# Improbable-AI/walk-these-ways

Hardware: AMD Instinct MI355X
Metric: env-steps/sec (sim+PPO) (higher is better)
Workload: dtype f32

## Files before the change

### walk-these-ways_amd/csrc/go1ppo_gemm.h

```cpp
#pragma once

#define GEMM_BM 128
#define GEMM_BN 128
#define GEMM_BK 64

typedef __attribute__((address_space(3))) void lds_void_t;
typedef __attribute__((address_space(1))) const void global_cvoid_t;

__device__ __forceinline__ void glds16(const bf16_t* g, bf16_t* lds_wave_base) {
  __builtin_amdgcn_global_load_lds((global_cvoid_t*)g, (lds_void_t*)lds_wave_base, 16, 0, 0);
}

template <int EPI>
__device__ __forceinline__ void gemm_nt_body(const Go1PpoGemmArgs& a, bf16_t (*lds)[2][GEMM_BM * GEMM_BK]) {
  const int lane = threadIdx.x & 63, wave = threadIdx.x >> 6;
  const int nwg = gridDim.x, orig = blockIdx.x;
  const int q = nwg >> 3, r = nwg & 7, xcd = orig & 7;
  const int logical = (xcd < r ? xcd * (q + 1) : r * (q + 1) + (xcd - r) * q) + (orig >> 3);
  const int tiles_n = (a.N + GEMM_BN - 1) / GEMM_BN;
  const int m0 = (logical / tiles_n) * GEMM_BM, n0 = (logical % tiles_n) * GEMM_BN;

  const int srow = lane >> 3;
  const bf16_t* ga[4];
  const bf16_t* gb[4];
#pragma unroll
  for (int p = 0; p < 4; p++) {
    int R = (wave * 4 + p) * 8 + srow;
    int chunk = (lane & 7) ^ ((R >> 1) & 7);
    int ra = m0 + R < a.M ? m0 + R : a.M - 1;
    int rb = n0 + R < a.N ? n0 + R : a.N - 1;
    ga[p] = (const bf16_t*)a.A + (int64_t)ra * a.lda + chunk * 8;
    gb[p] = (const bf16_t*)a.B + (int64_t)rb * a.ldb + chunk * 8;
  }
  auto stage = [&](int buf, int k0) {
#pragma unroll
    for (int p = 0; p < 4; p++) {
      glds16(ga[p] + k0, &lds[buf][0][(wave * 4 + p) * 8 * GEMM_BK]);
      glds16(gb[p] + k0, &lds[buf][1][(wave * 4 + p) * 8 * GEMM_BK]);
    }
  };

  const int fr = lane & 15, fg = lane >> 4;
  int foff[2];
#pragma unroll
  for (int kk = 0; kk < 2; kk++) foff[kk] = fr * GEMM_BK + (((kk * 4 + fg) ^ (fr >> 1)) << 3);
  const int wm = wave >> 1, wn = wave & 1;

  f32x4 acc[4][4];
#pragma unroll
  for (int i = 0; i < 4; i++)
#pragma unroll
    for (int j = 0; j < 4; j++) acc[i][j] = f32x4{0.f, 0.f, 0.f, 0.f};

  const bool wide = !(a.N & 7) && !(a.ldc & 7) && !((uintptr_t)a.C & 15) && (EPI != 2 || (!(a.ldh & 7) && !((uintptr_t)a.H & 15)));
  uint4 hrow[8];
  if (EPI == 2 && wide) {
#pragma unroll
    for (int it = 0; it < 8; it++) {
      int m = m0 + (int)(threadIdx.x >> 4) + 16 * it, n = n0 + (int)(threadIdx.x & 15) * 8;
      m = m < a.M ? m : a.M - 1;
      n = n < a.N ? n : a.N - 8;
      hrow[it] = *reinterpret_cast<const uint4*>((const bf16_t*)a.H + (int64_t)m * a.ldh + n);
    }
  }
  uint2 hpre[4][4];
  if (EPI == 2 && !wide) {
#pragma unroll
    for (int j = 0; j < 4; j++) {
      int n = n0 + wn * 64 + j * 16 + fg * 4;
      n = n < a.N ? n : a.N - 4;
#pragma unroll
      for (int i = 0; i < 4; i++) {
        int m = m0 + wm * 64 + i * 16 + fr;
        m = m < a.M ? m : a.M - 1;
        hpre[j][i] = *reinterpret_cast<const uint2*>((const bf16_t*)a.H + (int64_t)m * a.ldh + n);
      }
    }
  }
  const int KT = a.K / GEMM_BK;
  stage(0, 0);
  for (int kt = 0; kt < KT; kt++) {
    const int buf = kt & 1;
    asm volatile("s_waitcnt vmcnt(0)" ::: "memory");
    __syncthreads();
    if (kt + 1 < KT) stage(buf ^ 1, (kt + 1) * GEMM_BK);
    const bf16_t* la = &lds[buf][0][wm * 64 * GEMM_BK];
    const bf16_t* lb = &lds[buf][1][wn * 64 * GEMM_BK];
#pragma unroll
    for (int kk = 0; kk < 2; kk++) {
      bf16x8_t xa[4], wb[4];
#pragma unroll
      for (int i = 0; i < 4; i++) xa[i] = *reinterpret_cast<const bf16x8_t*>(la + i * 16 * GEMM_BK + foff[kk]);
#pragma unroll
      for (int j = 0; j < 4; j++) wb[j] = *reinterpret_cast<const bf16x8_t*>(lb + j * 16 * GEMM_BK + foff[kk]);
#pragma unroll
      for (int j = 0; j < 4; j++)
#pragma unroll
        for (int i = 0; i < 4; i++) acc[j][i] = __builtin_amdgcn_mfma_f32_16x16x32_bf16(wb[j], xa[i], acc[j][i], 0, 0, 0);
    }
  }

  if (wide) {
    __syncthreads();
    float* img = reinterpret_cast<float*>(&lds[0][0][0]);
#pragma unroll
    for (int j = 0; j < 4; j++) {
      const int nl = wn * 64 + j * 16 + fg * 4, n = n0 + nl;
      f32x4 bias = f32x4{0.f, 0.f, 0.f, 0.f};
      if (a.bias && n < a.N) {
        if (a.bias_bf16) {
          const uint2 braw = *reinterpret_cast<const uint2*>(reinterpret_cast<const bf16_t*>(a.bias) + n);
          bias = f32x4{__uint_as_float(braw.x << 16), __uint_as_float(braw.x & 0xffff0000u), __uint_as_float(braw.y << 16),
                       __uint_as_float(braw.y & 0xffff0000u)};
        } else bias = *reinterpret_cast<const f32x4*>(a.bias + n);
      }
      const bool act = EPI == 1 && n >= a.elu_c0 && n < a.elu_c1 && !(n >= a.elu_skip_c0 && n < a.elu_skip_c1);
#pragma unroll
      for (int i = 0; i < 4; i++) {
        const int row = wm * 64 + i * 16 + fr;
        f32x4 v = acc[j][i] + bias;
        if (act) {
#pragma unroll
          for (int e = 0; e < 4; e++) v[e] = elu1(v[e]);
        }
        *reinterpret_cast<f32x4*>(img + row * 128 + ((((nl >> 2)) ^ (row & 15)) << 2)) = v;
      }
    }
    __syncthreads();
    const int c8 = (int)(threadIdx.x & 15);
    const int n = n0 + c8 * 8;
#pragma unroll
    for (int it = 0; it < 8; it++) {
      const int row = (int)(threadIdx.x >> 4) + 16 * it, m = m0 + row;
      const f32x4 lo = *reinterpret_cast<const f32x4*>(img + row * 128 + (((2 * c8) ^ (row & 15)) << 2));
      const f32x4 hi = *reinterpret_cast<const f32x4*>(img + row * 128 + (((2 * c8 + 1) ^ (row & 15)) << 2));
      float v[8] = {lo[0], lo[1], lo[2], lo[3], hi[0], hi[1], hi[2], hi[3]};
      if (EPI == 2) {
        const uint32_t hw[4] = {hrow[it].x, hrow[it].y, hrow[it].z, hrow[it].w};
#pragma unroll
        for (int e = 0; e < 4; e++) {
          const float h0 = __uint_as_float(hw[e] << 16), h1 = __uint_as_float(hw[e] & 0xffff0000u);
          v[2 * e] *= h0 > 0.f ? 1.f : h0 + 1.f;
          v[2 * e + 1] *= h1 > 0.f ? 1.f : h1 + 1.f;
        }
      }
      if (m < a.M && n < a.N) {
        uint4 o;
        uint32_t* ow = reinterpret_cast<uint32_t*>(&o);
#pragma unroll
        for (int e = 0; e < 4; e++) {
          f32x2 p2 = {v[2 * e], v[2 * e + 1]};
          ow[e] = __builtin_bit_cast(uint32_t, __builtin_convertvector(p2, bf16x2_t));
        }
        *reinterpret_cast<uint4*>((bf16_t*)a.C + (int64_t)m * a.ldc + n) = o;
      }
    }
    return;
  }
#pragma unroll
  for (int j = 0; j < 4; j++) {
    const int n = n0 + wn * 64 + j * 16 + fg * 4;
    if (n >= a.N) continue;
    f32x4 bias = f32x4{0.f, 0.f, 0.f, 0.f};
    if (a.bias) {
      if (a.bias_bf16) {
        const uint2 braw = *reinterpret_cast<const uint2*>(reinterpret_cast<const bf16_t*>(a.bias) + n);
        bias = f32x4{__uint_as_float(braw.x << 16), __uint_as_float(braw.x & 0xffff0000u), __uint_as_float(braw.y << 16),
                     __uint_as_float(braw.y & 0xffff0000u)};
      } else bias = *reinterpret_cast<const f32x4*>(a.bias + n);
    }
#pragma unroll
    for (int i = 0; i < 4; i++) {
      const int m = m0 + wm * 64 + i * 16 + fr;
      if (m >= a.M) continue;
      float v[4];
#pragma unroll
      for (int e = 0; e < 4; e++) v[e] = acc[j][i][e] + bias[e];
      if (EPI == 1) {
        if (n >= a.elu_c0 && n < a.elu_c1 && !(n >= a.elu_skip_c0 && n < a.elu_skip_c1)) {
#pragma unroll
          for (int e = 0; e < 4; e++) v[e] = elu1(v[e]);
        }
      } else if (EPI == 2) {
        const uint2 hraw = hpre[j][i];
        float h[4] = {__uint_as_float(hraw.x << 16), __uint_as_float(hraw.x & 0xffff0000u), __uint_as_float(hraw.y << 16),
                      __uint_as_float(hraw.y & 0xffff0000u)};
#pragma unroll
        for (int e = 0; e < 4; e++) v[e] *= h[e] > 0.f ? 1.f : h[e] + 1.f;
      }
      f32x2 lo = {v[0], v[1]}, hi = {v[2], v[3]};
      uint2 o;
      o.x = __builtin_bit_cast(uint32_t, __builtin_convertvector(lo, bf16x2_t));
      o.y = __builtin_bit_cast(uint32_t, __builtin_convertvector(hi, bf16x2_t));
      *reinterpret_cast<uint2*>((bf16_t*)a.C + (int64_t)m * a.ldc + n) = o;
    }
  }
}

template <int EPI>
__global__ __launch_bounds__(256, 2) void gemm_nt_kernel(Go1PpoGemmArgs a) {
  __shared__ __attribute__((aligned(1024))) bf16_t lds[2][2][GEMM_BM * GEMM_BK];
  gemm_nt_body<EPI>(a, lds);
}
template <int EPI>
__global__ __launch_bounds__(256, 2) void gemm_nt_pair_kernel(Go1PpoGemmArgs a, Go1PpoGemmArgs b) {
  __shared__ __attribute__((aligned(1024))) bf16_t lds[2][2][GEMM_BM * GEMM_BK];
  gemm_nt_body<EPI>(blockIdx.y == 0 ? a : b, lds);
}

static int gemm_nt_check(const Go1PpoGemmArgs* a) {
  if (!a || !a->A || !a->B || !a->C || a->M <= 0 || a->N <= 0 || a->K <= 0) return -1;
  if ((a->K % GEMM_BK) || (a->N & 3) || (a->lda & 7) || (a->ldb & 7) || (a->ldc & 3) || !aligned16(a->A) || !aligned16(a->B) ||
      ((uintptr_t)a->C & 7))
    return -2;
  if (a->epilogue == 2 && (!a->H || (a->ldh & 3) || ((uintptr_t)a->H & 7))) return -3;
  if (a->bias && ((uintptr_t)a->bias & (a->bias_bf16 ? 7 : 15))) return -4;
  return 0;
}

extern "C" int go1ppo_gemm_nt_pair(const Go1PpoGemmArgs* a, const Go1PpoGemmArgs* b, void* stream) {
  int rc = gemm_nt_check(a);
  if (rc == 0) rc = gemm_nt_check(b);
  if (rc) return rc;
  const int64_t tiles = (int64_t)((a->M + GEMM_BM - 1) / GEMM_BM) * ((a->N + GEMM_BN - 1) / GEMM_BN);
  const int64_t tiles_b = (int64_t)((b->M + GEMM_BM - 1) / GEMM_BM) * ((b->N + GEMM_BN - 1) / GEMM_BN);
  if (tiles > INT32_MAX) return -5;
  if (tiles != tiles_b || a->epilogue != b->epilogue) return -7;
  dim3 grid((unsigned)tiles, 2), block(256);
  hipStream_t s = (hipStream_t)stream;
  switch (a->epilogue) {
    case 0: gemm_nt_pair_kernel<0><<<grid, block, 0, s>>>(*a, *b); break;
    case 1: gemm_nt_pair_kernel<1><<<grid, block, 0, s>>>(*a, *b); break;
    case 2: gemm_nt_pair_kernel<2><<<grid, block, 0, s>>>(*a, *b); break;
    default: return -6;
  }
  return hipGetLastError() == hipSuccess ? 0 : -9;
}

extern "C" int go1ppo_gemm_nt(const Go1PpoGemmArgs* a, void* stream) {
  const int rc = gemm_nt_check(a);
  if (rc) return rc;
  int64_t tiles = (int64_t)((a->M + GEMM_BM - 1) / GEMM_BM) * ((a->N + GEMM_BN - 1) / GEMM_BN);
  if (tiles > INT32_MAX) return -5;
  dim3 grid((unsigned)tiles), block(256);
  hipStream_t s = (hipStream_t)stream;
  switch (a->epilogue) {
    case 0: gemm_nt_kernel<0><<<grid, block, 0, s>>>(*a); break;
    case 1: gemm_nt_kernel<1><<<grid, block, 0, s>>>(*a); break;
    case 2: gemm_nt_kernel<2><<<grid, block, 0, s>>>(*a); break;
    default: return -6;
  }
  return hipGetLastError() == hipSuccess ? 0 : -9;
}

typedef __attribute__((ext_vector_type(4))) short s16x4_t;
typedef __attribute__((ext_vector_type(8))) short s16x8_t;
template <int OFF>
__device__ __forceinline__ s16x4_t lds_tr(uint32_t addr) {
  s16x4_t v;
  asm volatile("ds_read_b64_tr_b16 %0, %1 offset:%2" : "=v"(v) : "v"(addr), "n"(OFF));
  return v;
}
struct TnFrags { s16x4_t lo[6], hi[6]; };
template <int KK>
__device__ __forceinline__ void tn_read(TnFrags& f, const uint32_t (&aa)[4], const uint32_t (&ab)[2]) {
#pragma unroll
  for (int i = 0; i < 4; i++) {
    f.lo[i] = lds_tr<KK * 32 * 256>(aa[i]);
    f.hi[i] = lds_tr<KK * 32 * 256 + 4 * 256>(aa[i]);
  }
#pragma unroll
  for (int i = 0; i < 2; i++) {
    f.lo[4 + i] = lds_tr<KK * 32 * 256>(ab[i]);
    f.hi[4 + i] = lds_tr<KK * 32 * 256 + 4 * 256>(ab[i]);
  }
}
template <int N>
__device__ __forceinline__ void lds_wait(TnFrags& f) {
  asm volatile("s_waitcnt lgkmcnt(%12)"
               : "+v"(f.lo[0]), "+v"(f.hi[0]), "+v"(f.lo[1]), "+v"(f.hi[1]), "+v"(f.lo[2]), "+v"(f.hi[2]), "+v"(f.lo[3]), "+v"(f.hi[3]),
                 "+v"(f.lo[4]), "+v"(f.hi[4]), "+v"(f.lo[5]), "+v"(f.hi[5])
               : "n"(N));
}
__device__ __forceinline__ bf16x8_t tn_operand(const TnFrags& f, int i) {
  s16x8_t v = __builtin_shufflevector(f.lo[i], f.hi[i], 0, 1, 2, 3, 4, 5, 6, 7);
  return __builtin_bit_cast(bf16x8_t, v);
}

#define WTN_T 128
#define WTN_STEP 64
#define WTN_BUFS 4
#define WTN_THREADS 512

__device__ __forceinline__ bool wtn_rows_ok(bool slab, const float* C, int ldc) { return slab && !(ldc & 3) && !((uintptr_t)C & 15); }
__device__ __forceinline__ int wtn_img_chunk(int row, int chunk) { return chunk ^ (((row >> 2) & 3) << 2); }
__device__ __forceinline__ void wtn_img_put(float* img, int row, int col, float x) {
  img[row * WTN_T + (wtn_img_chunk(row, col >> 2) << 2) + (col & 3)] = x;
}
template <int ROWS>
__device__ __forceinline__ void wtn_slab_rows(const float* img, float* C, int ldc, int N, int K, int n0, int k0, int zero_n, int zero_k0,
                                              int zero_k1) {
  const int chunk = threadIdx.x & 31, k = k0 + 4 * chunk;
  if (k >= K) return;
#pragma unroll
  for (int it = 0; it < ROWS / (WTN_THREADS / 32); it++) {
    const int row = (int)(threadIdx.x >> 5) + (WTN_THREADS / 32) * it, n = n0 + row;
    if (n >= N) continue;
    const f32x4 v = *reinterpret_cast<const f32x4*>(img + row * WTN_T + (wtn_img_chunk(row, chunk) << 2));
    float* dst = C + (int64_t)n * ldc + k;
    if (!(n < zero_n && k < zero_k1 && k + 4 > zero_k0)) put16_wt(dst, v);
    else {
#pragma unroll
      for (int e = 0; e < 4; e++)
        if (!(k + e >= zero_k0 && k + e < zero_k1)) det_put(dst + e, v[e]);
    }
  }
}

__device__ __forceinline__ void wgrad_tn_body(const bf16_t* P, int ldp, const bf16_t* Q, int ldq, int64_t m_begin, int steps,
                                              float* C, int ldc, float* bias_row, int N, int K, int n0, int k0,
                                              bf16_t (*lds)[2][WTN_STEP * WTN_T], int zero_n, int zero_k0, int zero_k1, bool slab) {
  const int lane = threadIdx.x & 63, wave = threadIdx.x >> 6;
  const bf16_t* gp[2];
  const bf16_t* gq[2];
  bool vp[2], vq[2];
#pragma unroll
  for (int p = 0; p < 2; p++) {
    const int row = (wave * 2 + p) * 4 + (lane >> 4);
    const int chunk = (lane & 15) ^ (2 * ((row & 3) | (((row >> 3) & 1) << 2)));
    const int cn = n0 + chunk * 8, ck = k0 + chunk * 8;
    vp[p] = cn < N;
    vq[p] = ck < K;
    gp[p] = P + (m_begin + row) * ldp + (vp[p] ? cn : 0);
    gq[p] = Q + (m_begin + row) * ldq + (vq[p] ? ck : 0);
  }
  auto stage_piece = [&](int step, int p, int op) {
    const int buf = step & (WTN_BUFS - 1);
    if (op == 0) { if (vp[p]) glds16(gp[p] + (int64_t)step * WTN_STEP * ldp, &lds[buf][0][(wave * 2 + p) * 4 * WTN_T]); }
    else { if (vq[p]) glds16(gq[p] + (int64_t)step * WTN_STEP * ldq, &lds[buf][1][(wave * 2 + p) * 4 * WTN_T]); }
  };
  auto stage = [&](int step) {
    stage_piece(step, 0, 0); stage_piece(step, 0, 1); stage_piece(step, 1, 0); stage_piece(step, 1, 1);
  };
  const int g = lane >> 4, i16 = lane & 15;
  const int rowoff = (g * 8 + (i16 >> 2)) * 256 + ((i16 & 3) >> 1) * 16 + (i16 & 1) * 8;
  const int swb = 32 * ((i16 >> 2) | ((g & 1) << 2));
  const int wn = wave >> 2, wk = wave & 3;
  int fa[4], fb[2];
#pragma unroll
  for (int f = 0; f < 4; f++) fa[f] = rowoff + (((wn * 64 + f * 16) * 2) ^ swb);
#pragma unroll
  for (int f = 0; f < 2; f++) fb[f] = rowoff + (((wk * 32 + f * 16) * 2) ^ swb);
  f32x4 acc[4][2], bacc[4];
#pragma unroll
  for (int a = 0; a < 4; a++) {
    bacc[a] = f32x4{0.f, 0.f, 0.f, 0.f};
#pragma unroll
    for (int b = 0; b < 2; b++) acc[a][b] = f32x4{0.f, 0.f, 0.f, 0.f};
  }
  const bool do_bias = bias_row && k0 == 0 && wk == 0;
  const s16x8_t ones_bits = {0x3f80, 0x3f80, 0x3f80, 0x3f80, 0x3f80, 0x3f80, 0x3f80, 0x3f80};
  const bf16x8_t ones = __builtin_bit_cast(bf16x8_t, ones_bits);

  const uint32_t lds0 = (uint32_t)(uintptr_t)(lds_void_t*)&lds[0][0][0];
#pragma unroll
  for (int s = 0; s < WTN_BUFS - 1; s++)
    if (s < steps) stage(s);
  for (int s = 0; s < steps; s++) {
    const int younger = steps - 1 - s;
    if (younger >= 2) asm volatile("s_waitcnt vmcnt(8)" ::: "memory");
    else if (younger == 1) asm volatile("s_waitcnt vmcnt(4)" ::: "memory");
    else asm volatile("s_waitcnt vmcnt(0)" ::: "memory");
    __builtin_amdgcn_s_barrier();
    asm volatile("" ::: "memory");
    const bool more = s + WTN_BUFS - 1 < steps;
    const int nxt = s + WTN_BUFS - 1;
    const uint32_t base = lds0 + (uint32_t)(s & (WTN_BUFS - 1)) * (2 * WTN_STEP * WTN_T * 2);
    uint32_t aa[4], ab[2];
#pragma unroll
    for (int f = 0; f < 4; f++) aa[f] = base + fa[f];
#pragma unroll
    for (int f = 0; f < 2; f++) ab[f] = base + WTN_STEP * WTN_T * 2 + fb[f];
    TnFrags f0, f1;
    tn_read<0>(f0, aa, ab);
    tn_read<1>(f1, aa, ab);
    if (more) { stage_piece(nxt, 0, 0); stage_piece(nxt, 0, 1); }
    lds_wait<12>(f0);
#pragma unroll
    for (int a = 0; a < 4; a++) {
#pragma unroll
      for (int b = 0; b < 2; b++)
        acc[a][b] = __builtin_amdgcn_mfma_f32_16x16x32_bf16(tn_operand(f0, a), tn_operand(f0, 4 + b), acc[a][b], 0, 0, 0);
      if (a == 1 && more) stage_piece(nxt, 1, 0);
    }
    if (do_bias) {
#pragma unroll
      for (int a = 0; a < 4; a++) bacc[a] = __builtin_amdgcn_mfma_f32_16x16x32_bf16(tn_operand(f0, a), ones, bacc[a], 0, 0, 0);
    }
    if (more) stage_piece(nxt, 1, 1);
    lds_wait<0>(f1);
#pragma unroll
    for (int a = 0; a < 4; a++)
#pragma unroll
      for (int b = 0; b < 2; b++)
        acc[a][b] = __builtin_amdgcn_mfma_f32_16x16x32_bf16(tn_operand(f1, a), tn_operand(f1, 4 + b), acc[a][b], 0, 0, 0);
    if (do_bias) {
#pragma unroll
      for (int a = 0; a < 4; a++) bacc[a] = __builtin_amdgcn_mfma_f32_16x16x32_bf16(tn_operand(f1, a), ones, bacc[a], 0, 0, 0);
    }
  }
  if (wtn_rows_ok(slab, C, ldc)) {
    float* img = reinterpret_cast<float*>(&lds[0][0][0]);
    __syncthreads();
#pragma unroll
    for (int a = 0; a < 4; a++)
#pragma unroll
      for (int e = 0; e < 4; e++)
#pragma unroll
        for (int b = 0; b < 2; b++) wtn_img_put(img, wn * 64 + a * 16 + 4 * g + e, wk * 32 + b * 16 + i16, acc[a][b][e]);
    __syncthreads();
    wtn_slab_rows<WTN_T>(img, C, ldc, N, K, n0, k0, zero_n, zero_k0, zero_k1);
  }
#pragma unroll
  for (int a = 0; a < 4; a++) {
#pragma unroll
    for (int e = 0; e < 4; e++) {
      const int n = n0 + wn * 64 + a * 16 + 4 * g + e;
      if (n >= N || wtn_rows_ok(slab, C, ldc)) continue;
#pragma unroll
      for (int b = 0; b < 2; b++) {
        const int k = k0 + wk * 32 + b * 16 + i16;
        if (k < K && !(n < zero_n && k >= zero_k0 && k < zero_k1)) {
          if (slab) C[(int64_t)n * ldc + k] = acc[a][b][e];
          else atomicAdd(C + (int64_t)n * ldc + k, acc[a][b][e]);
        }
      }
    }
    if (do_bias && i16 == 0 && n0 + wn * 64 + a * 16 + 4 * g < N) det_put4(bias_row, (wn * 64 + a * 16 + 4 * g) * (int)sizeof(float), bacc[a]);
  }
}

#define WTW_BUF_BYTES (3 * WTN_STEP * WTN_T * 2)
#define WTW_BUFS 3
struct TnFragsW { s16x4_t lo[8], hi[8]; };
template <int KK>
__device__ __forceinline__ void tnw_read(TnFragsW& f, const uint32_t (&aa)[4], const uint32_t (&ab)[4]) {
#pragma unroll
  for (int i = 0; i < 4; i++) {
    f.lo[i] = lds_tr<KK * 32 * 256>(aa[i]);
    f.hi[i] = lds_tr<KK * 32 * 256 + 4 * 256>(aa[i]);
  }
#pragma unroll
  for (int i = 0; i < 4; i++) {
    f.lo[4 + i] = lds_tr<KK * 32 * 256>(ab[i]);
    f.hi[4 + i] = lds_tr<KK * 32 * 256 + 4 * 256>(ab[i]);
  }
}
__device__ __forceinline__ void ldsw_wait_all(TnFragsW& f) {
  asm volatile("s_waitcnt lgkmcnt(0)"
               : "+v"(f.lo[0]), "+v"(f.lo[1]), "+v"(f.lo[2]), "+v"(f.lo[3]), "+v"(f.lo[4]), "+v"(f.lo[5]), "+v"(f.lo[6]), "+v"(f.lo[7]));
  asm volatile("" : "+v"(f.hi[0]), "+v"(f.hi[1]), "+v"(f.hi[2]), "+v"(f.hi[3]), "+v"(f.hi[4]), "+v"(f.hi[5]), "+v"(f.hi[6]), "+v"(f.hi[7]));
}
__device__ __forceinline__ bf16x8_t tnw_operand(const TnFragsW& f, int i) {
  s16x8_t v = __builtin_shufflevector(f.lo[i], f.hi[i], 0, 1, 2, 3, 4, 5, 6, 7);
  return __builtin_bit_cast(bf16x8_t, v);
}

__device__ __forceinline__ void wgrad_tn_body_wide(const bf16_t* P, int ldp, const bf16_t* Q, int ldq, int64_t m_begin, int steps,
                                                   float* C, int ldc, float* bias_row, int N, int K, int n0, int k0, char* lds,
                                                   int zero_n, int zero_k0, int zero_k1, bool slab) {
  const int lane = threadIdx.x & 63, wave = threadIdx.x >> 6;
  const bf16_t* src[6];
  bool ok[6];
  int dst[6];
#pragma unroll
  for (int q = 0; q < 6; q++) {
    const int id = q < 4 ? wave * 4 + q : wave * 2 + (q - 4);
    const int img = q < 4 ? id >> 4 : 2, rb = q < 4 ? id & 15 : id;
    const int row = rb * 4 + (lane >> 4);
    const int chunk = (lane & 15) ^ (2 * ((row & 3) | (((row >> 3) & 1) << 2)));
    const int col = (q < 4 ? n0 + img * 128 : k0) + chunk * 8;
    ok[q] = col < (q < 4 ? N : K);
    src[q] = (q < 4 ? P + (m_begin + row) * ldp : Q + (m_begin + row) * ldq) + (ok[q] ? col : 0);
    dst[q] = img * (WTN_STEP * WTN_T * 2) + rb * 4 * WTN_T * 2;
  }
  auto stage_piece = [&](int step, int buf, int q) {
    if (ok[q]) glds16(src[q] + (int64_t)step * WTN_STEP * (q < 4 ? ldp : ldq), (bf16_t*)(lds + buf * WTW_BUF_BYTES + dst[q]));
  };
  const int g = lane >> 4, i16 = lane & 15;
  const int rowoff = (g * 8 + (i16 >> 2)) * 256 + ((i16 & 3) >> 1) * 16 + (i16 & 1) * 8;
  const int swb = 32 * ((i16 >> 2) | ((g & 1) << 2));
  const int wn = wave >> 1, wk = wave & 1;
  int fa[4], fb[4];
#pragma unroll
  for (int f = 0; f < 4; f++) {
    fa[f] = (wn >> 1) * (WTN_STEP * WTN_T * 2) + rowoff + ((((wn & 1) * 64 + f * 16) * 2) ^ swb);
    fb[f] = 2 * (WTN_STEP * WTN_T * 2) + rowoff + (((wk * 64 + f * 16) * 2) ^ swb);
  }
  f32x4 acc[4][4], bacc[4];
#pragma unroll
  for (int a = 0; a < 4; a++) {
    bacc[a] = f32x4{0.f, 0.f, 0.f, 0.f};
#pragma unroll
    for (int b = 0; b < 4; b++) acc[a][b] = f32x4{0.f, 0.f, 0.f, 0.f};
  }
  const bool do_bias = bias_row && k0 == 0 && wk == 0;
  const s16x8_t ones_bits = {0x3f80, 0x3f80, 0x3f80, 0x3f80, 0x3f80, 0x3f80, 0x3f80, 0x3f80};
  const bf16x8_t ones = __builtin_bit_cast(bf16x8_t, ones_bits);
  const uint32_t lds0 = (uint32_t)(uintptr_t)(lds_void_t*)lds;
#pragma unroll
  for (int s = 0; s < WTW_BUFS - 1; s++)
    if (s < steps) {
#pragma unroll
      for (int q = 0; q < 6; q++) stage_piece(s, s, q);
    }
  int buf = 0;
  for (int s = 0; s < steps; s++) {
    if (s + 1 < steps) asm volatile("s_waitcnt vmcnt(6)" ::: "memory");
    else asm volatile("s_waitcnt vmcnt(0)" ::: "memory");
    __builtin_amdgcn_s_barrier();
    asm volatile("" ::: "memory");
    const bool more = s + WTW_BUFS - 1 < steps;
    const int nxt = s + WTW_BUFS - 1, nbuf = buf == 0 ? WTW_BUFS - 1 : buf - 1;
    const uint32_t base = lds0 + (uint32_t)buf * WTW_BUF_BYTES;
    uint32_t aa[4], ab[4];
#pragma unroll
    for (int f = 0; f < 4; f++) { aa[f] = base + fa[f]; ab[f] = base + fb[f]; }
    TnFragsW f0, f1;
    tnw_read<0>(f0, aa, ab);
    if (more) { stage_piece(nxt, nbuf, 0); stage_piece(nxt, nbuf, 1); stage_piece(nxt, nbuf, 4); }
    ldsw_wait_all(f0);
    tnw_read<1>(f1, aa, ab);
#pragma unroll
    for (int a = 0; a < 4; a++) {
#pragma unroll
      for (int b = 0; b < 4; b++)
        acc[a][b] = __builtin_amdgcn_mfma_f32_16x16x32_bf16(tnw_operand(f0, a), tnw_operand(f0, 4 + b), acc[a][b], 0, 0, 0);
      if (more && a < 3) stage_piece(nxt, nbuf, a == 0 ? 2 : (a == 1 ? 3 : 5));
    }
    if (do_bias) {
#pragma unroll
      for (int a = 0; a < 4; a++) bacc[a] = __builtin_amdgcn_mfma_f32_16x16x32_bf16(tnw_operand(f0, a), ones, bacc[a], 0, 0, 0);
    }
    ldsw_wait_all(f1);
#pragma unroll
    for (int a = 0; a < 4; a++)
#pragma unroll
      for (int b = 0; b < 4; b++)
        acc[a][b] = __builtin_amdgcn_mfma_f32_16x16x32_bf16(tnw_operand(f1, a), tnw_operand(f1, 4 + b), acc[a][b], 0, 0, 0);
    if (do_bias) {
#pragma unroll
      for (int a = 0; a < 4; a++) bacc[a] = __builtin_amdgcn_mfma_f32_16x16x32_bf16(tnw_operand(f1, a), ones, bacc[a], 0, 0, 0);
// ... 127 lines not shown
```

Measured before the change: 5.250 million.

## Make NT GEMM persistent with 3-stage pipelined LDS loads and adaptive tile height

Rewrites the NT bf16 GEMM as a persistent kernel that launches at most one 512-thread workgroup per CU and walks several tiles. Global-to-LDS copies run through a 3-stage ring with fine-grained vmcnt waits, and copies for the next step are interleaved with the MFMA work. A separate LDS region holds the epilogue image, so the next tile's prefetch can continue across tile boundaries. A 64-row tile is chosen when the problem has too few tiles to fill the CUs, and H/bias loads are prefetched with inline asm. In exchange, occupancy drops to one workgroup per CU and LDS use is larger.

```diff
diff --git a/walk-these-ways_amd/csrc/go1ppo_gemm.h b/walk-these-ways_amd/csrc/go1ppo_gemm.h
--- a/walk-these-ways_amd/csrc/go1ppo_gemm.h
+++ b/walk-these-ways_amd/csrc/go1ppo_gemm.h
@@ -3,6 +3,10 @@
 #define GEMM_BM 128
 #define GEMM_BN 128
 #define GEMM_BK 64
+#define GEMM_STAGES 3
+#define GEMM_THREADS 512
+#define GEMM_STAGE_BYTES ((GEMM_BM + GEMM_BN) * GEMM_BK * 2)
+#define GEMM_CUS 256
 
 typedef __attribute__((address_space(3))) void lds_void_t;
 typedef __attribute__((address_space(1))) const void global_cvoid_t;
@@ -10,202 +14,324 @@
 __device__ __forceinline__ void glds16(const bf16_t* g, bf16_t* lds_wave_base) {
   __builtin_amdgcn_global_load_lds((global_cvoid_t*)g, (lds_void_t*)lds_wave_base, 16, 0, 0);
 }
-
-template <int EPI>
-__device__ __forceinline__ void gemm_nt_body(const Go1PpoGemmArgs& a, bf16_t (*lds)[2][GEMM_BM * GEMM_BK]) {
+template <int OFF>
+__device__ __forceinline__ u32x4_t lds_rd16(uint32_t addr) {
+  u32x4_t v;
+  asm volatile("ds_read_b128 %0, %1 offset:%2" : "=v"(v) : "v"(addr), "n"(OFF));
+  return v;
+}
+template <int MI>
+struct NtFrags { u32x4_t x[MI], w[2]; };
+template <int MI, int KK>
+__device__ __forceinline__ void nt_read(NtFrags<MI>& f, uint32_t ax, uint32_t aw) {
+  f.x[0] = lds_rd16<0>(ax);
+  f.x[1] = lds_rd16<16 * GEMM_BK * 2>(ax);
+  if constexpr (MI == 4) {
+    f.x[2] = lds_rd16<32 * GEMM_BK * 2>(ax);
+    f.x[3] = lds_rd16<48 * GEMM_BK * 2>(ax);
+  }
+  f.w[0] = lds_rd16<GEMM_BM * GEMM_BK * 2>(aw);
+  f.w[1] = lds_rd16<GEMM_BM * GEMM_BK * 2 + 16 * GEMM_BK * 2>(aw);
+}
+template <int N, int MI>
+__device__ __forceinline__ void nt_wait(NtFrags<MI>& f) {
+  if constexpr (MI == 4)
+    asm volatile("s_waitcnt lgkmcnt(%6)" : "+v"(f.x[0]), "+v"(f.x[1]), "+v"(f.x[2]), "+v"(f.x[3]), "+v"(f.w[0]), "+v"(f.w[1]) : "n"(N));
+  else
+    asm volatile("s_waitcnt lgkmcnt(%4)" : "+v"(f.x[0]), "+v"(f.x[1]), "+v"(f.w[0]), "+v"(f.w[1]) : "n"(N));
+}
+template <int PER_STEP>
+__device__ __forceinline__ void nt_wait_dma(int younger) {
+  if (younger >= 3) asm volatile("s_waitcnt vmcnt(%0)" ::"n"(3 * PER_STEP) : "memory");
+  else if (younger == 2) asm volatile("s_waitcnt vmcnt(%0)" ::"n"(2 * PER_STEP) : "memory");
+  else if (younger == 1) asm volatile("s_waitcnt vmcnt(%0)" ::"n"(PER_STEP) : "memory");
+  else asm volatile("s_waitcnt vmcnt(0)" ::: "memory");
+}
+
+__device__ __forceinline__ u32x4_t gload16(const void* p) {
+  u32x4_t v;
+  asm volatile("global_load_dwordx4 %0, %1, off" : "=v"(v) : "v"(p));
+  return v;
+}
+typedef __attribute__((ext_vector_type(2))) uint32_t u32x2_t;
+__device__ __forceinline__ u32x2_t gload8(const void* p) {
+  u32x2_t v;
+  asm volatile("global_load_dwordx2 %0, %1, off" : "=v"(v) : "v"(p));
+  return v;
+}
+
+__device__ __forceinline__ bool gemm_nt_wide(const Go1PpoGemmArgs& a) {
+  return !(a.N & 7) && !(a.ldc & 7) && !((uintptr_t)a.C & 15) && (a.epilogue != 2 || (!(a.ldh & 7) && !((uintptr_t)a.H & 15)));
+}
+
+template <int EPI, int BM, bool WIDE>
+__device__ __forceinline__ void gemm_nt_body(const Go1PpoGemmArgs& a, char* lds) {
+  constexpr int AP = BM / 64;
+  constexpr int NPS = AP + 2;
+  constexpr int MI = BM / 32;
+  constexpr int IT = BM / 32;
   const int lane = threadIdx.x & 63, wave = threadIdx.x >> 6;
-  const int nwg = gridDim.x, orig = blockIdx.x;
-  const int q = nwg >> 3, r = nwg & 7, xcd = orig & 7;
-  const int logical = (xcd < r ? xcd * (q + 1) : r * (q + 1) + (xcd - r) * q) + (orig >> 3);
-  const int tiles_n = (a.N + GEMM_BN - 1) / GEMM_BN;
-  const int m0 = (logical / tiles_n) * GEMM_BM, n0 = (logical % tiles_n) * GEMM_BN;
+  const int tiles_n = (a.N + GEMM_BN - 1) / GEMM_BN, tiles = ((a.M + BM - 1) / BM) * tiles_n;
+  const int nwg = gridDim.x, xcd = blockIdx.x & 7, slot = blockIdx.x >> 3;
+  const int q = tiles >> 3, r = tiles & 7;
+  const int first = (xcd < r ? xcd * (q + 1) : r * (q + 1) + (xcd - r) * q) + slot, mine = q + (xcd < r) - slot;
+  const int slots = (nwg >> 3) + (xcd < (nwg & 7));
+  if (mine <= 0) return;
+  const int ntiles = (mine + slots - 1) / slots;
 
   const int srow = lane >> 3;
-  const bf16_t* ga[4];
-  const bf16_t* gb[4];
-#pragma unroll
-  for (int p = 0; p < 4; p++) {
-    int R = (wave * 4 + p) * 8 + srow;
-    int chunk = (lane & 7) ^ ((R >> 1) & 7);
-    int ra = m0 + R < a.M ? m0 + R : a.M - 1;
-    int rb = n0 + R < a.N ? n0 + R : a.N - 1;
-    ga[p] = (const bf16_t*)a.A + (int64_t)ra * a.lda + chunk * 8;
-    gb[p] = (const bf16_t*)a.B + (int64_t)rb * a.ldb + chunk * 8;
-  }
-  auto stage = [&](int buf, int k0) {
-#pragma unroll
-    for (int p = 0; p < 4; p++) {
-      glds16(ga[p] + k0, &lds[buf][0][(wave * 4 + p) * 8 * GEMM_BK]);
-      glds16(gb[p] + k0, &lds[buf][1][(wave * 4 + p) * 8 * GEMM_BK]);
+  const int KT = a.K / GEMM_BK, steps = ntiles * KT;
+  const bf16_t* ga[AP];
+  const bf16_t* gb[2];
+  int i_tile = 0, i_kt = 0, i_buf = 0, issued = 0;
+  auto stage_begin = [&]() {
+    if (i_kt != 0) return;
+    const int logical = first + i_tile * slots;
+    const int m0 = (logical / tiles_n) * BM, n0 = (logical % tiles_n) * GEMM_BN;
+#pragma unroll
+    for (int p = 0; p < AP; p++) {
+      int R = (wave * AP + p) * 8 + srow;
+      int chunk = (lane & 7) ^ ((R >> 1) & 7);
+      int ra = m0 + R < a.M ? m0 + R : a.M - 1;
+      ga[p] = (const bf16_t*)a.A + (int64_t)ra * a.lda + chunk * 8;
+    }
+#pragma unroll
+    for (int p = 0; p < 2; p++) {
+      int R = (wave * 2 + p) * 8 + srow;
+      int chunk = (lane & 7) ^ ((R >> 1) & 7);
+      int rb = n0 + R < a.N ? n0 + R : a.N - 1;
+      gb[p] = (const bf16_t*)a.B + (int64_t)rb * a.ldb + chunk * 8;
     }
   };
+  auto stage_piece = [&](int piece) {
+    char* dst = lds + i_buf * GEMM_STAGE_BYTES;
+    if (piece < AP) glds16(ga[piece] + i_kt * GEMM_BK, (bf16_t*)(dst + (wave * AP + piece) * 8 * GEMM_BK * 2));
+    else glds16(gb[piece - AP] + i_kt * GEMM_BK, (bf16_t*)(dst + GEMM_BM * GEMM_BK * 2 + (wave * 2 + piece - AP) * 8 * GEMM_BK * 2));
+  };
+  auto stage_end = [&]() {
+    issued++;
+    i_buf = i_buf + 1 == GEMM_STAGES ? 0 : i_buf + 1;
+    if (++i_kt == KT) { i_kt = 0; i_tile++; }
+  };
 
   const int fr = lane & 15, fg = lane >> 4;
-  int foff[2];
-#pragma unroll
-  for (int kk = 0; kk < 2; kk++) foff[kk] = fr * GEMM_BK + (((kk * 4 + fg) ^ (fr >> 1)) << 3);
-  const int wm = wave >> 1, wn = wave & 1;
-
-  f32x4 acc[4][4];
-#pragma unroll
-  for (int i = 0; i < 4; i++)
-#pragma unroll
-    for (int j = 0; j < 4; j++) acc[i][j] = f32x4{0.f, 0.f, 0.f, 0.f};
-
-  const bool wide = !(a.N & 7) && !(a.ldc & 7) && !((uintptr_t)a.C & 15) && (EPI != 2 || (!(a.ldh & 7) && !((uintptr_t)a.H & 15)));
-  uint4 hrow[8];
-  if (EPI == 2 && wide) {
-#pragma unroll
-    for (int it = 0; it < 8; it++) {
-      int m = m0 + (int)(threadIdx.x >> 4) + 16 * it, n = n0 + (int)(threadIdx.x & 15) * 8;
-      m = m < a.M ? m : a.M - 1;
-      n = n < a.N ? n : a.N - 8;
-      hrow[it] = *reinterpret_cast<const uint4*>((const bf16_t*)a.H + (int64_t)m * a.ldh + n);
-    }
-  }
-  uint2 hpre[4][4];
-  if (EPI == 2 && !wide) {
-#pragma unroll
-    for (int j = 0; j < 4; j++) {
-      int n = n0 + wn * 64 + j * 16 + fg * 4;
-      n = n < a.N ? n : a.N - 4;
-#pragma unroll
-      for (int i = 0; i < 4; i++) {
-        int m = m0 + wm * 64 + i * 16 + fr;
-        m = m < a.M ? m : a.M - 1;
-        hpre[j][i] = *reinterpret_cast<const uint2*>((const bf16_t*)a.H + (int64_t)m * a.ldh + n);
-      }
-    }
-  }
-  const int KT = a.K / GEMM_BK;
-  stage(0, 0);
-  for (int kt = 0; kt < KT; kt++) {
-    const int buf = kt & 1;
-    asm volatile("s_waitcnt vmcnt(0)" ::: "memory");
-    __syncthreads();
-    if (kt + 1 < KT) stage(buf ^ 1, (kt + 1) * GEMM_BK);
-    const bf16_t* la = &lds[buf][0][wm * 64 * GEMM_BK];
-    const bf16_t* lb = &lds[buf][1][wn * 64 * GEMM_BK];
-#pragma unroll
-    for (int kk = 0; kk < 2; kk++) {
-      bf16x8_t xa[4], wb[4];
-#pragma unroll
-      for (int i = 0; i < 4; i++) xa[i] = *reinterpret_cast<const bf16x8_t*>(la + i * 16 * GEMM_BK + foff[kk]);
-#pragma unroll
-      for (int j = 0; j < 4; j++) wb[j] = *reinterpret_cast<const bf16x8_t*>(lb + j * 16 * GEMM_BK + foff[kk]);
-#pragma unroll
-      for (int j = 0; j < 4; j++)
-#pragma unroll
-        for (int i = 0; i < 4; i++) acc[j][i] = __builtin_amdgcn_mfma_f32_16x16x32_bf16(wb[j], xa[i], acc[j][i], 0, 0, 0);
-    }
-  }
-
-  if (wide) {
-    __syncthreads();
-    float* img = reinterpret_cast<float*>(&lds[0][0][0]);
-#pragma unroll
-    for (int j = 0; j < 4; j++) {
-      const int nl = wn * 64 + j * 16 + fg * 4, n = n0 + nl;
+  const int wm = wave >> 2, wn = wave & 3;
+  const uint32_t lds0 = (uint32_t)(uintptr_t)(lds_void_t*)lds;
+  uint32_t fx[2], fw[2];
+#pragma unroll
+  for (int kk = 0; kk < 2; kk++) {
+    const int foff = (fr * GEMM_BK + (((kk * 4 + fg) ^ (fr >> 1)) << 3)) * 2;
+    fx[kk] = lds0 + wm * (BM / 2) * GEMM_BK * 2 + foff;
+    fw[kk] = lds0 + wn * 32 * GEMM_BK * 2 + foff;
+  }
+  float* img = reinterpret_cast<float*>(lds + GEMM_STAGES * GEMM_STAGE_BYTES);
+  const uint32_t img0 = lds0 + GEMM_STAGES * GEMM_STAGE_BYTES;
+
+  for (int s = steps <= GEMM_STAGES ? steps : GEMM_STAGES - 1; s > 0; s--) {
+    stage_begin();
+#pragma unroll
+    for (int p = 0; p < NPS; p++) stage_piece(p);
+    stage_end();
+  }
+  int c_buf = 0, done = 0;
+  for (int t = 0; t < ntiles; t++) {
+    const int logical = first + t * slots;
+    const int m0 = (logical / tiles_n) * BM, n0 = (logical % tiles_n) * GEMM_BN;
+    u32x4_t hrow[IT] = {}, bias4[2] = {};
+    u32x2_t bias2[2] = {};
+    int since = 0;
+    if (WIDE) {
+      if (EPI == 2) {
+#pragma unroll
+        for (int it = 0; it < IT; it++) {
+          int m = m0 + (int)(threadIdx.x >> 4) + 32 * it, n = n0 + (int)(threadIdx.x & 15) * 8;
+          m = m < a.M ? m : a.M - 1;
+          n = n < a.N ? n : a.N - 8;
+          hrow[it] = gload16((const bf16_t*)a.H + (int64_t)m * a.ldh + n);
+        }
+      }
+      if (a.bias) {
+#pragma unroll
+        for (int j = 0; j < 2; j++) {
+          int n = n0 + wn * 32 + j * 16 + fg * 4;
+          n = n < a.N ? n : 0;
+          if (a.bias_bf16) bias2[j] = gload8(reinterpret_cast<const bf16_t*>(a.bias) + n);
+          else bias4[j] = gload16(a.bias + n);
+        }
+      }
+    }
+    f32x4 acc[2][MI];
+#pragma unroll
+    for (int j = 0; j < 2; j++)
+#pragma unroll
+      for (int i = 0; i < MI; i++) acc[j][i] = f32x4{0.f, 0.f, 0.f, 0.f};
+
+    for (int kt = 0; kt < KT; kt++) {
+      nt_wait_dma<NPS>(issued - 1 - done);
+      __builtin_amdgcn_s_barrier();
+      asm volatile("" ::: "memory");
+      const bool more = issued < steps;
+      const uint32_t base = (uint32_t)c_buf * GEMM_STAGE_BYTES;
+      NtFrags<MI> f0, f1;
+      nt_read<MI, 0>(f0, base + fx[0], base + fw[0]);
+      nt_read<MI, 1>(f1, base + fx[1], base + fw[1]);
+      if (more) {
+        stage_begin();
+#pragma unroll
+        for (int p = 0; p < AP; p++) stage_piece(p);
+      }
+      nt_wait<MI + 2>(f0);
+#pragma unroll
+      for (int j = 0; j < 2; j++) {
+#pragma unroll
+        for (int i = 0; i < MI; i++)
+          acc[j][i] = __builtin_amdgcn_mfma_f32_16x16x32_bf16(__builtin_bit_cast(bf16x8_t, f0.w[j]), __builtin_bit_cast(bf16x8_t, f0.x[i]), acc[j][i], 0, 0, 0);
+        if (more) stage_piece(AP + j);
+      }
+      nt_wait<0>(f1);
+#pragma unroll
+      for (int j = 0; j < 2; j++)
+#pragma unroll
+        for (int i = 0; i < MI; i++)
+          acc[j][i] = __builtin_amdgcn_mfma_f32_16x16x32_bf16(__builtin_bit_cast(bf16x8_t, f1.w[j]), __builtin_bit_cast(bf16x8_t, f1.x[i]), acc[j][i], 0, 0, 0);
+      if (more) { stage_end(); since++; }
+      c_buf = c_buf + 1 == GEMM_STAGES ? 0 : c_buf + 1;
+      done++;
+    }
+
+    if constexpr (WIDE) {
+      nt_wait_dma<NPS>(since < GEMM_STAGES - 1 ? since : GEMM_STAGES - 1);
+      if (EPI == 2) {
+#pragma unroll
+        for (int it = 0; it < IT; it++) asm volatile("" : "+v"(hrow[it]));
+      }
+      asm volatile("" : "+v"(bias4[0]), "+v"(bias4[1]), "+v"(bias2[0]), "+v"(bias2[1]));
+#pragma unroll
+      for (int j = 0; j < 2; j++) {
+        const int nl = wn * 32 + j * 16 + fg * 4, n = n0 + nl;
+        f32x4 bias = f32x4{0.f, 0.f, 0.f, 0.f};
+        if (a.bias) {
+          if (a.bias_bf16)
+            bias = f32x4{__uint_as_float(bias2[j].x << 16), __uint_as_float(bias2[j].x & 0xffff0000u), __uint_as_float(bias2[j].y << 16),
+                         __uint_as_float(bias2[j].y & 0xffff0000u)};
+          else bias = __builtin_bit_cast(f32x4, bias4[j]);
+        }
+        const bool act = EPI == 1 && n >= a.elu_c0 && n < a.elu_c1 && !(n >= a.elu_skip_c0 && n < a.elu_skip_c1);
+#pragma unroll
+        for (int i = 0; i < MI; i++) {
+          const int row = wm * (BM / 2) + i * 16 + fr;
+          f32x4 v = acc[j][i] + bias;
+          if (act) {
+#pragma unroll
+            for (int e = 0; e < 4; e++) v[e] = elu1(v[e]);
+          }
+          *reinterpret_cast<f32x4*>(img + row * 128 + ((((nl >> 2)) ^ (row & 15)) << 2)) = v;
+        }
+      }
+      asm volatile("s_waitcnt lgkmcnt(0)" ::: "memory");
+      __builtin_amdgcn_s_barrier();
+      asm volatile("" ::: "memory");
+      const int c8 = (int)(threadIdx.x & 15);
+      const int n = n0 + c8 * 8;
+      u32x4_t lo[IT], hi[IT];
+#pragma unroll
+      for (int it = 0; it < IT; it++) {
+        const int row = (int)(threadIdx.x >> 4) + 32 * it;
+        lo[it] = lds_rd16<0>(img0 + (row * 128 + (((2 * c8) ^ (row & 15)) << 2)) * 4);
+        hi[it] = lds_rd16<0>(img0 + (row * 128 + (((2 * c8 + 1) ^ (row & 15)) << 2)) * 4);
+      }
+      if constexpr (IT == 4)
+        asm volatile("s_waitcnt lgkmcnt(0)" : "+v"(lo[0]), "+v"(hi[0]), "+v"(lo[1]), "+v"(hi[1]), "+v"(lo[2]), "+v"(hi[2]), "+v"(lo[3]), "+v"(hi[3]));
+      else
+        asm volatile("s_waitcnt lgkmcnt(0)" : "+v"(lo[0]), "+v"(hi[0]), "+v"(lo[1]), "+v"(hi[1]));
+#pragma unroll
+      for (int it = 0; it < IT; it++) {
+        const int m = m0 + (int)(threadIdx.x >> 4) + 32 * it;
+        const f32x4 l4 = __builtin_bit_cast(f32x4, lo[it]), h4 = __builtin_bit_cast(f32x4, hi[it]);
+        float v[8] = {l4[0], l4[1], l4[2], l4[3], h4[0], h4[1], h4[2], h4[3]};
+        if (EPI == 2) {
+          const uint32_t hw[4] = {hrow[it].x, hrow[it].y, hrow[it].z, hrow[it].w};
+#pragma unroll
+          for (int e = 0; e < 4; e++) {
+            const float h0 = __uint_as_float(hw[e] << 16), h1 = __uint_as_float(hw[e] & 0xffff0000u);
+            v[2 * e] *= h0 > 0.f ? 1.f : h0 + 1.f;
+            v[2 * e + 1] *= h1 > 0.f ? 1.f : h1 + 1.f;
+          }
+        }
+        if (m < a.M && n < a.N) {
+          uint4 o;
+          uint32_t* ow = reinterpret_cast<uint32_t*>(&o);
+#pragma unroll
+          for (int e = 0; e < 4; e++) {
+            f32x2 p2 = {v[2 * e], v[2 * e + 1]};
+            ow[e] = __builtin_bit_cast(uint32_t, __builtin_convertvector(p2, bf16x2_t));
+          }
+          *reinterpret_cast<uint4*>((bf16_t*)a.C + (int64_t)m * a.ldc + n) = o;
+        }
+      }
+    } else {
+#pragma unroll
+    for (int j = 0; j < 2; j++) {
+      const int n = n0 + wn * 32 + j * 16 + fg * 4;
+      if (n >= a.N) continue;
       f32x4 bias = f32x4{0.f, 0.f, 0.f, 0.f};
-      if (a.bias && n < a.N) {
+      if (a.bias) {
         if (a.bias_bf16) {
           const uint2 braw = *reinterpret_cast<const uint2*>(reinterpret_cast<const bf16_t*>(a.bias) + n);
           bias = f32x4{__uint_as_float(braw.x << 16), __uint_as_float(braw.x & 0xffff0000u), __uint_as_float(braw.y << 16),
                        __uint_as_float(braw.y & 0xffff0000u)};
         } else bias = *reinterpret_cast<const f32x4*>(a.bias + n);
       }
-      const bool act = EPI == 1 && n >= a.elu_c0 && n < a.elu_c1 && !(n >= a.elu_skip_c0 && n < a.elu_skip_c1);
-#pragma unroll
-      for (int i = 0; i < 4; i++) {
-        const int row = wm * 64 + i * 16 + fr;
-        f32x4 v = acc[j][i] + bias;
-        if (act) {
-#pragma unroll
-          for (int e = 0; e < 4; e++) v[e] = elu1(v[e]);
+#pragma unroll
+      for (int i = 0; i < MI; i++) {
+        const int m = m0 + wm * (BM / 2) + i * 16 + fr;
+        if (m >= a.M) continue;
+        float v[4];
+#pragma unroll
+        for (int e = 0; e < 4; e++) v[e] = acc[j][i][e] + bias[e];
+        if (EPI == 1) {
+          if (n >= a.elu_c0 && n < a.elu_c1 && !(n >= a.elu_skip_c0 && n < a.elu_skip_c1)) {
+#pragma unroll
+            for (int e = 0; e < 4; e++) v[e] = elu1(v[e]);
+          }
+        } else if (EPI == 2) {
+          const uint2 hraw = *reinterpret_cast<const uint2*>((const bf16_t*)a.H + (int64_t)m * a.ldh + n);
+          float h[4] = {__uint_as_float(hraw.x << 16), __uint_as_float(hraw.x & 0xffff0000u), __uint_as_float(hraw.y << 16),
+                        __uint_as_float(hraw.y & 0xffff0000u)};
+#pragma unroll
+          for (int e = 0; e < 4; e++) v[e] *= h[e] > 0.f ? 1.f : h[e] + 1.f;
         }
-        *reinterpret_cast<f32x4*>(img + row * 128 + ((((nl >> 2)) ^ (row & 15)) << 2)) = v;
-      }
-    }
-    __syncthreads();
-    const int c8 = (int)(threadIdx.x & 15);
-    const int n = n0 + c8 * 8;
-#pragma unroll
-    for (int it = 0; it < 8; it++) {
-      const int row = (int)(threadIdx.x >> 4) + 16 * it, m = m0 + row;
-      const f32x4 lo = *reinterpret_cast<const f32x4*>(img + row * 128 + (((2 * c8) ^ (row & 15)) << 2));
-      const f32x4 hi = *reinterpret_cast<const f32x4*>(img + row * 128 + (((2 * c8 + 1) ^ (row & 15)) << 2));
-      float v[8] = {lo[0], lo[1], lo[2], lo[3], hi[0], hi[1], hi[2], hi[3]};
-      if (EPI == 2) {
-        const uint32_t hw[4] = {hrow[it].x, hrow[it].y, hrow[it].z, hrow[it].w};
-#pragma unroll
-        for (int e = 0; e < 4; e++) {
-          const float h0 = __uint_as_float(hw[e] << 16), h1 = __uint_as_float(hw[e] & 0xffff0000u);
-          v[2 * e] *= h0 > 0.f ? 1.f : h0 + 1.f;
-          v[2 * e + 1] *= h1 > 0.f ? 1.f : h1 + 1.f;
-        }
-      }
-      if (m < a.M && n < a.N) {
-        uint4 o;
-        uint32_t* ow = reinterpret_cast<uint32_t*>(&o);
-#pragma unroll
-        for (int e = 0; e < 4; e++) {
-          f32x2 p2 = {v[2 * e], v[2 * e + 1]};
-          ow[e] = __builtin_bit_cast(uint32_t, __builtin_convertvector(p2, bf16x2_t));
-        }
-        *reinterpret_cast<uint4*>((bf16_t*)a.C + (int64_t)m * a.ldc + n) = o;
-      }
-    }
-    return;
-  }
-#pragma unroll
-  for (int j = 0; j < 4; j++) {
-    const int n = n0 + wn * 64 + j * 16 + fg * 4;
-    if (n >= a.N) continue;
-    f32x4 bias = f32x4{0.f, 0.f, 0.f, 0.f};
-    if (a.bias) {
-      if (a.bias_bf16) {
-        const uint2 braw = *reinterpret_cast<const uint2*>(reinterpret_cast<const bf16_t*>(a.bias) + n);
-        bias = f32x4{__uint_as_float(braw.x << 16), __uint_as_float(braw.x & 0xffff0000u), __uint_as_float(braw.y << 16),
-                     __uint_as_float(braw.y & 0xffff0000u)};
-      } else bias = *reinterpret_cast<const f32x4*>(a.bias + n);
-    }
-#pragma unroll
-    for (int i = 0; i < 4; i++) {
-      const int m = m0 + wm * 64 + i * 16 + fr;
-      if (m >= a.M) continue;
-      float v[4];
-#pragma unroll
-      for (int e = 0; e < 4; e++) v[e] = acc[j][i][e] + bias[e];
-      if (EPI == 1) {
-        if (n >= a.elu_c0 && n < a.elu_c1 && !(n >= a.elu_skip_c0 && n < a.elu_skip_c1)) {
-#pragma unroll
-          for (int e = 0; e < 4; e++) v[e] = elu1(v[e]);
-        }
-      } else if (EPI == 2) {
-        const uint2 hraw = hpre[j][i];
-        float h[4] = {__uint_as_float(hraw.x << 16), __uint_as_float(hraw.x & 0xffff0000u), __uint_as_float(hraw.y << 16),
-                      __uint_as_float(hraw.y & 0xffff0000u)};
-#pragma unroll
-        for (int e = 0; e < 4; e++) v[e] *= h[e] > 0.f ? 1.f : h[e] + 1.f;
-      }
-      f32x2 lo = {v[0], v[1]}, hi = {v[2], v[3]};
-      uint2 o;
-      o.x = __builtin_bit_cast(uint32_t, __builtin_convertvector(lo, bf16x2_t));
-      o.y = __builtin_bit_cast(uint32_t, __builtin_convertvector(hi, bf16x2_t));
-      *reinterpret_cast<uint2*>((bf16_t*)a.C + (int64_t)m * a.ldc + n) = o;
-    }
-  }
-}
-
+        f32x2 lo = {v[0], v[1]}, hi = {v[2], v[3]};
+        uint2 o;
+        o.x = __builtin_bit_cast(uint32_t, __builtin_convertvector(lo, bf16x2_t));
+        o.y = __builtin_bit_cast(uint32_t, __builtin_convertvector(hi, bf16x2_t));
+        *reinterpret_cast<uint2*>((bf16_t*)a.C + (int64_t)m * a.ldc + n) = o;
+      }
+    }
+    }
+  }
+}
 template <int EPI>
-__global__ __launch_bounds__(256, 2) void gemm_nt_kernel(Go1PpoGemmArgs a) {
-  __shared__ __attribute__((aligned(1024))) bf16_t lds[2][2][GEMM_BM * GEMM_BK];
-  gemm_nt_body<EPI>(a, lds);
-}
+__device__ __forceinline__ void gemm_nt_tile(const Go1PpoGemmArgs& a, char* lds, int small) {
+  if (gemm_nt_wide(a)) {
+    if (small) gemm_nt_body<EPI, GEMM_BM / 2, true>(a, lds);
+    else gemm_nt_body<EPI, GEMM_BM, true>(a, lds);
+  } else {
+    if (small) gemm_nt_body<EPI, GEMM_BM / 2, false>(a, lds);
+    else gemm_nt_body<EPI, GEMM_BM, false>(a, lds);
+  }
+}
+
+#define GEMM_LDS_BYTES (GEMM_STAGES * GEMM_STAGE_BYTES + GEMM_BM * GEMM_BN * 4)
 template <int EPI>
-__global__ __launch_bounds__(256, 2) void gemm_nt_pair_kernel(Go1PpoGemmArgs a, Go1PpoGemmArgs b) {
-  __shared__ __attribute__((aligned(1024))) bf16_t lds[2][2][GEMM_BM * GEMM_BK];
-  gemm_nt_body<EPI>(blockIdx.y == 0 ? a : b, lds);
+__global__ __launch_bounds__(GEMM_THREADS, 1) void gemm_nt_kernel(Go1PpoGemmArgs a, int small) {
+  __shared__ __attribute__((aligned(1024))) char lds[GEMM_LDS_BYTES];
+  gemm_nt_tile<EPI>(a, lds, small);
+}
+template <int EPI>
+__global__ __launch_bounds__(GEMM_THREADS, 1) void gemm_nt_pair_kernel(Go1PpoGemmArgs a, Go1PpoGemmArgs b, int small) {
+  __shared__ __attribute__((aligned(1024))) char lds[GEMM_LDS_BYTES];
+  gemm_nt_tile<EPI>(blockIdx.y == 0 ? a : b, lds, small);
 }
 
 static int gemm_nt_check(const Go1PpoGemmArgs* a) {
@@ -217,21 +343,26 @@
   if (a->bias && ((uintptr_t)a->bias & (a->bias_bf16 ? 7 : 15))) return -4;
   return 0;
 }
+static int64_t gemm_nt_tiles(const Go1PpoGemmArgs* a, int rows) {
+  return (int64_t)((a->M + rows - 1) / rows) * ((a->N + GEMM_BN - 1) / GEMM_BN);
+}
+static int gemm_nt_tile_rows(int64_t tiles64, int problems) { return tiles64 * problems <= GEMM_CUS ? GEMM_BM / 2 : GEMM_BM; }
 
 extern "C" int go1ppo_gemm_nt_pair(const Go1PpoGemmArgs* a, const Go1PpoGemmArgs* b, void* stream) {
   int rc = gemm_nt_check(a);
   if (rc == 0) rc = gemm_nt_check(b);
   if (rc) return rc;
-  const int64_t tiles = (int64_t)((a->M + GEMM_BM - 1) / GEMM_BM) * ((a->N + GEMM_BN - 1) / GEMM_BN);
-  const int64_t tiles_b = (int64_t)((b->M + GEMM_BM - 1) / GEMM_BM) * ((b->N + GEMM_BN - 1) / GEMM_BN);
-  if (tiles > INT32_MAX) return -5;
-  if (tiles != tiles_b || a->epilogue != b->epilogue) return -7;
-  dim3 grid((unsigned)tiles, 2), block(256);
+  if (gemm_nt_tiles(a, GEMM_BM) > INT32_MAX) return -5;
+  if (gemm_nt_tiles(a, GEMM_BM) != gemm_nt_tiles(b, GEMM_BM) || a->epilogue != b->epilogue) return -7;
+  const int64_t t64a = gemm_nt_tiles(a, GEMM_BM / 2), t64b = gemm_nt_tiles(b, GEMM_BM / 2);
+  const int rows = gemm_nt_tile_rows(t64a > t64b ? t64a : t64b, 2), small = rows != GEMM_BM;
+  const int64_t tiles = small ? (t64a > t64b ? t64a : t64b) : gemm_nt_tiles(a, GEMM_BM);
+  dim3 grid((unsigned)(tiles < GEMM_CUS / 2 ? tiles : GEMM_CUS / 2), 2), block(GEMM_THREADS);
   hipStream_t s = (hipStream_t)stream;
   switch (a->epilogue) {
-    case 0: gemm_nt_pair_kernel<0><<<grid, block, 0, s>>>(*a, *b); break;
-    case 1: gemm_nt_pair_kernel<1><<<grid, block, 0, s>>>(*a, *b); break;
-    case 2: gemm_nt_pair_kernel<2><<<grid, block, 0, s>>>(*a, *b); break;
+    case 0: gemm_nt_pair_kernel<0><<<grid, block, 0, s>>>(*a, *b, small); break;
+    case 1: gemm_nt_pair_kernel<1><<<grid, block, 0, s>>>(*a, *b, small); break;
+    case 2: gemm_nt_pair_kernel<2><<<grid, block, 0, s>>>(*a, *b, small); break;
     default: return -6;
   }
   return hipGetLastError() == hipSuccess ? 0 : -9;
@@ -240,14 +371,15 @@
 extern "C" int go1ppo_gemm_nt(const Go1PpoGemmArgs* a, void* stream) {
   const int rc = gemm_nt_check(a);
   if (rc) return rc;
-  int64_t tiles = (int64_t)((a->M + GEMM_BM - 1) / GEMM_BM) * ((a->N + GEMM_BN - 1) / GEMM_BN);
-  if (tiles > INT32_MAX) return -5;
-  dim3 grid((unsigned)tiles), block(256);
+  if (gemm_nt_tiles(a, GEMM_BM) > INT32_MAX) return -5;
+  const int rows = gemm_nt_tile_rows(gemm_nt_tiles(a, GEMM_BM / 2), 1), small = rows != GEMM_BM;
+  const int64_t tiles = gemm_nt_tiles(a, rows);
+  dim3 grid((unsigned)(tiles < GEMM_CUS ? tiles : GEMM_CUS)), block(GEMM_THREADS);
   hipStream_t s = (hipStream_t)stream;
   switch (a->epilogue) {
-    case 0: gemm_nt_kernel<0><<<grid, block, 0, s>>>(*a); break;
-    case 1: gemm_nt_kernel<1><<<grid, block, 0, s>>>(*a); break;
-    case 2: gemm_nt_kernel<2><<<grid, block, 0, s>>>(*a); break;
+    case 0: gemm_nt_kernel<0><<<grid, block, 0, s>>>(*a, small); break;
+    case 1: gemm_nt_kernel<1><<<grid, block, 0, s>>>(*a, small); break;
+    case 2: gemm_nt_kernel<2><<<grid, block, 0, s>>>(*a, small); break;
     default: return -6;
   }
   return hipGetLastError() == hipSuccess ? 0 : -9;
```

Result: no change. 5.269 million, median of 3 (+0.4%).
